# jzombie/rust-simd-r-drive

Hardware: AMD Instinct MI355X
Metric: GiB/s hashed (device-resident), full-file validate+index scan (higher is better)
Workload: dtype u8

## Files before the change

include/srd_amd.h:

```cpp
#ifndef SRD_AMD_H
#define SRD_AMD_H
#include <stddef.h>
#include <stdint.h>

#ifdef __cplusplus
extern "C" {
#endif

#define SRD_OK 0
#define SRD_ERR_HIP (-1)
#define SRD_ERR_ALLOC (-2)
#define SRD_ERR_ARG (-3)
#define SRD_ERR_INTERNAL (-4)

#define SRD_MODE_OPTIMISTIC 0
#define SRD_MODE_FULL 1
#define SRD_MODE_SPAN_UNPROVEN 3

#define SRD_FULL_NONE 0
#define SRD_FULL_FORCED 1
#define SRD_FULL_SLOT_SPACE 2
#define SRD_FULL_WAVES 3
#define SRD_FULL_NO_START 4
#define SRD_FULL_UNPROVEN 5
#define SRD_FULL_CAP 6
#define SRD_FULL_LOOKBACK 7

#define SRD_FLAG_FORCE_FULL 1u
#define SRD_FLAG_NO_CRC 2u
#define SRD_FLAG_STAGE_PAGEABLE 4u
#define SRD_FLAG_STAGE_REGISTER 8u

typedef struct srd_ctx srd_ctx;

int srd_ctx_create(int device, srd_ctx **out);
void srd_ctx_destroy(srd_ctx *ctx);
void *srd_ctx_stream(srd_ctx *ctx);
uint64_t srd_ctx_device_bytes(srd_ctx *ctx);
int srd_ctx_scan_loads(srd_ctx *ctx);
int srd_ctx_scan_trial(srd_ctx *ctx, double *ms);
#define SRD_SCAN_BLOCKS_LAST 0
#define SRD_SCAN_BLOCKS_NEXT 1
#define SRD_SCAN_BLOCKS_EVEN 0
#define SRD_SCAN_BLOCKS_MEASURED 1
#define SRD_SCAN_BLOCKS_INSTALLED 2
typedef struct {
  uint64_t n_spans;
  uint32_t n_blocks;
  uint32_t source;
  uint32_t attempts;
  uint32_t first_source;
} srd_scan_blocks_info;
int srd_ctx_set_scan_blocks(srd_ctx *ctx, const uint64_t *starts,
                            uint32_t n_blocks, uint64_t n_spans);
int srd_ctx_scan_blocks(srd_ctx *ctx, int which, uint64_t *starts,
                        uint32_t cap, srd_scan_blocks_info *info);
const char *srd_last_error(void);
const char *srd_build_info(void);
#define SRD_TIMING_NONE 0
#define SRD_TIMING_SCAN 1
#define SRD_TIMING_CALL 2
int srd_ctx_set_timing(srd_ctx *ctx, int level);
// ... 324 lines not shown
```

rust-simd-r-drive_amd/csrc/srd_ctx.hip:

```cpp
static thread_local std::string g_err;
static void set_err(const std::string& s) { g_err = s; }

#define HIPCHK(x)                                                                         \
  do {                                                                                    \
    hipError_t e_ = (x);                                                                  \
    if (e_ != hipSuccess) {                                                               \
      set_err(std::string(#x) + ": " + hipGetErrorString(e_));                            \
      return SRD_ERR_HIP;                                                                 \
    }                                                                                     \
  } while (0)

namespace {

#define TRY(x)                 \
  do {                         \
    int r_ = (x);              \
    if (r_) return r_;         \
  } while (0)

static int launched(hipStream_t s, const char* name) {
  static const bool sync = [] { const char* e = getenv("SRD_SYNC_DEBUG"); return e && *e && *e != '0'; }();
  HIPCHK(hipGetLastError());
  if (!sync) return 0;
  hipError_t e = hipStreamSynchronize(s);
// ... 48 lines not shown
  }
  void post(std::function<void()> f) {
    std::lock_guard<std::mutex> lk(mu);
    job = std::move(f);
    has = true;
    cv.notify_all();
  }
  void wait() {
    std::unique_lock<std::mutex> lk(mu);
    cv.wait(lk, [this] { return !has; });
  }
};

struct Ctx {
  int device = 0;
  hipStream_t stream = nullptr;
  std::vector<Buf> bufs;
  CandCap copt{8, 8, 0, 8};
  CandCap cfull{32, 32, 0, 32};
  unsigned scan_blocks = 256;
  unsigned scan_cus = 256;
  uint32_t scan_wq[16] = {};
  uint32_t scan_variant = 0;
  uint64_t slot_limit = 1ull << 31;
  int loads_pin = -1;
  int last_loads = -1;
  struct LoadTune {
    uint64_t ns = ~0ull;
    uint32_t g = 0;
    uint32_t calls = 0;
    uint64_t best[2] = {0, 0};
    uint32_t n[2] = {0, 0};
    int choice = -1;
  } tune;
  bool glue_fused = true;
  uint32_t lb_fail = ~0u;
  bool xpart_on = true, xp_valid = false;
  uint32_t xp_par = 0, xp_g = 0;
  uint64_t xp_ns = 0;
  bool xp_installed = false;
  struct LastPart {
    bool any = false;
    uint64_t ns = 0;
    uint32_t g = 0, src = 0, par = 0;
    uint32_t attempts = 0, first_src = 0;
  } xp_last;
// ... 299 lines not shown
      gs += x;
      q = *end == ',' ? end + 1 : end;
      if (*end && *end != ',') { n = 0; break; }
    }
    if (!std::isfinite(gs)) n = 0;
    if (n == 4)
      for (int v = 0; v < 16; v++) f[v] = g[v / 4];
    else if (n == 16)
      for (int v = 0; v < 16; v++) f[v] = g[v];
  }
  weights_to_shares(f, wq);
}
#ifdef SRD_DEBUG_API
extern "C" int srd_debug_set_scan_variant(srd_ctx* c, int v) {
  if (!c || !(v == 0 || v == 7 || v == 8 || v == SCAN_LINES)) return SRD_ERR_ARG;
  c->scan_variant = (uint32_t)v;
  return 0;
}
extern "C" int srd_debug_set_scan_bpc(srd_ctx* c, int bpc) {
  if (!c || bpc < 1 || bpc > 2) return SRD_ERR_ARG;
  c->scan_blocks = c->scan_cus * (unsigned)bpc;
  return 0;
}
extern "C" int srd_debug_set_xpart(srd_ctx* c, int on) {
  if (!c) return SRD_ERR_ARG;
  c->xpart_on = on != 0;
  return 0;
}
extern "C" int srd_debug_set_glue_fused(srd_ctx* c, int fused) {
  if (!c) return SRD_ERR_ARG;
  c->glue_fused = fused != 0;
  return 0;
}
extern "C" int srd_debug_set_scan_weights(srd_ctx* c, const double* w, int n) {
  if (!c || !w || (n != 4 && n != 16)) return SRD_ERR_ARG;
  double f[16], sum = 0;
  for (int v = 0; v < 16; v++) {
    sum += f[v] = n == 4 ? w[v / 4] : w[v];
    if (!(f[v] > 0) || !std::isfinite(f[v])) return SRD_ERR_ARG;
  }
  if (!std::isfinite(sum)) return SRD_ERR_ARG;
  weights_to_shares(f, c->scan_wq);
  return 0;
}
#endif
static int ctx_init(srd_ctx* c, int device) {
// ... 2 lines not shown
  if (hipStreamCreateWithFlags(&c->stream, hipStreamNonBlocking) != hipSuccess) {
    set_err("hipStreamCreate failed");
    return SRD_ERR_HIP;
  }
  TRY(upload_tables());
  for (auto& e : c->ev) HIPCHK(hipEventCreateWithFlags(&e, hipEventReleaseToDevice));
  HIPCHK(hipEventCreateWithFlags(&c->ev_ready, hipEventDisableTiming));
  HIPCHK(hipHostMalloc((void**)&c->h_plan, sizeof(Plan), hipHostMallocDefault));
  HIPCHK(hipHostMalloc((void**)&c->h_pub, 64, hipHostMallocCoherent));
  memset(c->h_pub, 0, 64);
  HIPCHK(hipHostMalloc((void**)&c->h_small, 256, hipHostMallocDefault));
  c->stage_workers = (int)std::max(1u, std::min(8u, std::thread::hardware_concurrency()));
  int ncu = 0;
  if (hipDeviceGetAttribute(&ncu, hipDeviceAttributeMultiprocessorCount, device) == hipSuccess && ncu > 0)
    c->scan_cus = c->scan_blocks = (unsigned)ncu;
  scan_weights(c->scan_wq);
  if (const char* e = getenv("SRD_SLOT_LIMIT_LOG2")) {
    const long v = strtol(e, nullptr, 10);
    if (v >= 10 && v <= 31) c->slot_limit = 1ull << v;
  }
  if (const char* e = getenv("SRD_SCAN_LOADS")) {
    if (!strcmp(e, "lines")) c->loads_pin = SCAN_LINES;
    else if (!strcmp(e, "coal")) c->loads_pin = 0;
  }
  if (const char* e = getenv("SRD_GLUE_FUSED")) c->glue_fused = strcmp(e, "0") != 0;
  if (const char* e = getenv("SRD_XPART")) c->xpart_on = strcmp(e, "0") != 0;
  if (const char* e = getenv("SRD_LB_FAIL_BLOCK")) {
    char* end = nullptr;
    const unsigned long v = strtoul(e, &end, 10);
    if (end != e && v < CHAIN_BLOCKS) c->lb_fail = (uint32_t)v;
  }
  return 0;
}

extern "C" int srd_ctx_create(int device, srd_ctx** out) {
  if (!out) { set_err("null out"); return SRD_ERR_ARG; }
  int n = 0;
  HIPCHK(hipGetDeviceCount(&n));
  if (device < 0 || device >= n) { set_err("bad device index"); return SRD_ERR_ARG; }
  HIPCHK(hipSetDevice(device));
  auto* c = new srd_ctx();
  const int r = ctx_init(c, device);
  if (r) {
    srd_ctx_destroy(c);
    return r;
  }
// ... 15 lines not shown
    if (e) hipEventDestroy(e);
  if (c->h_plan) hipHostFree(c->h_plan);
  if (c->h_pub) hipHostFree(c->h_pub);
  if (c->h_small) hipHostFree(c->h_small);
  if (c->h_out) hipHostFree(c->h_out);
  for (int i = 0; i < 2; i++) {
    if (c->pin_ent[i]) hipHostFree(c->pin_ent[i]);
    if (c->wev_copied[i]) hipEventDestroy(c->wev_copied[i]);
    if (c->wev_done[i]) hipEventDestroy(c->wev_done[i]);
  }
  if (c->cstream) hipStreamDestroy(c->cstream);
  for (auto p : c->stage_pin)
    if (p) hipHostFree(p);
  for (auto e : c->stage_ev)
    if (e) hipEventDestroy(e);
  for (auto st : c->stage_streams)
    if (st) hipStreamDestroy(st);
  if (c->stream) hipStreamDestroy(c->stream);
  delete c;
}

extern "C" void* srd_ctx_stream(srd_ctx* c) { return c ? (void*)c->stream : nullptr; }
extern "C" int srd_ctx_scan_loads(srd_ctx* c) { return c ? c->last_loads : -1; }
extern "C" int srd_ctx_scan_trial(srd_ctx* c, double* ms) {
  if (!c) return -1;
  if (ms)
    for (int k = 0; k < 2; k++) ms[k] = c->tune.n[k] ? (double)c->tune.best[k] * 1e-5 : 0.0;
  return c->tune.choice;
}
extern "C" int srd_ctx_set_scan_blocks(srd_ctx* c, const uint64_t* starts, uint32_t n_blocks, uint64_t n_spans) {
  if (!c || !starts) { set_err("bad argument"); return SRD_ERR_ARG; }
  if (!c->xpart_on) { set_err("XCD-aware block shares are off on this context (SRD_XPART=0)"); return SRD_ERR_ARG; }
  if (!part_table_ok(starts, n_blocks, n_spans)) {
    set_err("bad argument: not a block-start table of n_blocks blocks over n_spans spans (srd_ctx_set_scan_blocks)");
    return SRD_ERR_ARG;
  }
  HIPCHK(hipSetDevice(c->device));
  TRY(ensure_z(c, B_XPART, sizeof(XPart)));
  HIPCHK(hipMemcpyAsync(&P<XPart>(c, B_XPART)->bs[c->xp_par][0], starts, ((size_t)n_blocks + 1) * 8,
                        hipMemcpyHostToDevice, c->stream));
  HIPCHK(hipStreamSynchronize(c->stream));
  c->xp_valid = true;
  c->xp_installed = true;
  c->xp_ns = n_spans;
  c->xp_g = n_blocks;
  return 0;
// ... 81 lines not shown
```

rust-simd-r-drive_amd/csrc/srd_glue.hip:

```cpp
#pragma once

namespace srd {

#define GST(ptr, val) srd_gst(&(ptr), (val))

struct Plan {
  uint64_t K;
  uint64_t n_chain;
  uint64_t root_t;
  uint64_t start;
  uint64_t n_index;
  uint64_t n_bad;
  uint64_t n_slow;
  uint64_t chain_core;
  uint64_t max_root, top_gap, overflow;
  uint32_t status;
  uint32_t nroot;
  uint32_t troot;
  uint32_t idx_overflow;
  uint32_t idx_alias;
};
constexpr uint32_t ST_NOSTART = 1, ST_SHAPE = 2, ST_ROOTS = 4, ST_OVERFLOW = 16;
constexpr uint64_t NO_NODE = ~0ull;

// ... 588 lines not shown
      if (!FUSED) pl->start = start;
      pl->status = s2;
      pl->chain_core = tot;
      pl->n_chain = s2 ? 0 : a.coff + tot;
    }
  };
  const bool plan_block = FUSED ? blockIdx.x + 1 == gridDim.x : blockIdx.x == 0;
  if (!FUSED && plan_block && threadIdx.x == 0) write_plan(st, total);
  if (FUSED && troot && plan_block && threadIdx.x == 0) write_plan(0, 0);
  if (st && !troot) return;
  __shared__ uint32_t s_vcnt[BW_MAX];
  __shared__ uint64_t s_lb[2];
  __shared__ uint32_t s_fail, s_nroot, s_lbok;
  __shared__ unsigned long long s_root_t;
  if constexpr (FUSED) {
    if (!troot) {
      if (threadIdx.x == 0) { s_fail = 0; s_nroot = 0; s_root_t = 0; }
      __syncthreads();
      const uint64_t tag = (uint64_t)a.gen << 32;
      const uint32_t wi = threadIdx.x >> 6, lane = threadIdx.x & 63;
      uint32_t nr = 0;
      bool fail = false;
      constexpr int CR = 4;
      for (uint32_t v = wi; v < a.wpb; v += CHAIN_WAVES) {
        const uint64_t w = (uint64_t)blockIdx.x * a.wpb + v;
        const uint32_t n = w < a.n_waves ? (uint32_t)min(a.wave_total[w] & ~(1ull << 63), a.wcap) : 0u;
        const uint64_t gb = w * a.wcap;
        int64_t c_par = PAR_MISS;
        uint64_t c_cg = 0;
        uint32_t cnt = 0;
        for (uint32_t base = 0; base < n; base += CR * 64) {
          uint64_t g[CR], cg[CR], cp[CR];
          int64_t par[CR], pp[CR];
          bool in[CR], need[CR];
#pragma unroll
          for (int r = 0; r < CR; r++) {
            const uint32_t i = base + (uint32_t)r * 64 + lane;
            in[r] = i < n;
            g[r] = gb + (in[r] ? i : 0u);
            par[r] = a.d_par[g[r]];
            cg[r] = a.childof[g[r]];
          }
          bool any = false;
#pragma unroll
          for (int r = 0; r < CR; r++) {
            const uint32_t i = base + (uint32_t)r * 64 + lane;
            const int64_t l0p = r ? (int64_t)(int32_t)__builtin_amdgcn_readlane((uint32_t)par[r - 1], 63) : c_par;
// ... 83 lines not shown
  }
  if (!FUSED || troot) {
    for (uint32_t k = threadIdx.x; k < nbk; k += blockDim.x) hist[k] = 0;
    fin_lds_words(lt, threadIdx.x, ltw, true);
    __syncthreads();
  }
  GLUE_STAMP(3);
  bool root_slow = false;
  const bool root_block = FUSED && !troot ? root_t != 0 : blockIdx.x == 0;
  if (root_block && a.coff && threadIdx.x == 0) {
    uint64_t kh;
    root_slow = finalize_core<true>(f, 0, NO_REC, -1, root_t, &kh, lt);
    atomicAdd(&hist[idx_bucket(kh, log2_nbk)], 1u);
  }
  uint64_t bend = a.coff + before;
  if (!troot) {
    const uint32_t wi = threadIdx.x >> 6, lane = threadIdx.x & 63;
    const uint64_t lt_mask = (1ull << lane) - 1;
    SlowQueue sq = {wslow[wi], 0, 0};
    if constexpr (FUSED) {
      uint32_t btot = 0;
      for (uint32_t v = 0; v < a.wpb; v++) btot += s_vcnt[v];
      bend += btot;
      for (uint32_t v = wi; v < a.wpb; v += CHAIN_WAVES) {
        const uint64_t w = (uint64_t)blockIdx.x * a.wpb + v;
        const uint32_t n = w < a.n_waves ? (uint32_t)min(a.wave_total[w] & ~(1ull << 63), a.wcap) : 0u;
        const uint64_t gb = w * a.wcap;
        uint32_t voff = 0;
        for (uint32_t u = 0; u < v; u++) voff += s_vcnt[u];
        uint64_t run = a.coff + before + voff;
        sq.run0 = run;
        uint32_t c_fl = F_NO_PARENT, c_suf = 0;
        for (uint32_t base = 0; base < n; base += 64 * FIN_R) {
          bool fl[FIN_R];
          uint64_t gi[FIN_R], kh[FIN_R];
          int64_t par[FIN_R];
          uint32_t psuf[FIN_R], rank[FIN_R];
          FinIn e[FIN_R];
#pragma unroll
          for (int r = 0; r < FIN_R; r++) {
            const uint32_t i = base + (uint32_t)r * 64 + lane;
            gi[r] = gb + (i < n ? i : 0u);
            fl[r] = fin_load_record(a, f, gi[r], i < n, e[r], kh[r], par[r], psuf[r]);
          }
          const uint32_t tot = fin_rank(fl, lt_mask, rank);
          bool any = false, need[FIN_R];
#pragma unroll
// ... 448 lines not shown
```

rust-simd-r-drive_amd/csrc/srd_kernels.hip:

```cpp
#include <hip/hip_runtime.h>
#include <stdint.h>

#include "srd_crc.h"
#include "srd_xxh3.h"
#include "srd_part.h"
#include "srd_fin.h"

namespace srd {


typedef uint32_t u32x4 __attribute__((ext_vector_type(4)));
typedef uint64_t u64x2 __attribute__((ext_vector_type(2)));
typedef uint16_t u16x2 __attribute__((ext_vector_type(2)));

constexpr int SPAN_TILES = 4;
constexpr uint64_t SPAN_BYTES = (uint64_t)TILE * SPAN_TILES;
constexpr int64_t PAR_ROOT = -1;
constexpr int64_t PAR_MISS = -2;

constexpr uint32_t F_NT = 256u, F_ZB = 512u;

struct DevTables {
  uint32_t tab[4][256];
  uint32_t lw[64];
// ... 333 lines not shown
  } else {
    const uint64_t wt = a.wave_total[w - 1] & ~(1ull << 63);
    hp = wt > 0 && wt <= a.wcap;
    gprev = (w - 1) * a.wcap + (hp ? wt - 1 : 0);
  }
  const bool hp2 = r >= 2;
  const uint64_t m = a.c_m[gi], mprev = hp ? a.c_m[gprev] : 0, mprev2 = hp2 ? a.c_m[gi - 2] : 0;
  const u32x4 r0 = a.c_rec[gi];
  const uint64_t p = (uint64_t)r0[0] | ((uint64_t)r0[1] << 32);
  bool node = true, tomb = false;
  if (r0[2] & F_NT) {
    const uint64_t dp = m - p;
    tomb = dp == 1 && (r0[2] & F_ZB);
    node = p >= 20 && p < m && (tomb || dp > prepad64(p));
  }
  const uint64_t mp = p - 20;
  const uint64_t sp2 = (mp + 14) / SPAN_BYTES;
  int64_t par = hp && mprev == mp ? (int64_t)gprev : hp2 && mprev2 == mp ? (int64_t)(gi - 2) : PAR_MISS;
  uint64_t pp = 1;
  const bool res = mp >= a.k_lo * (uint64_t)TILE;
  if (node && par == PAR_MISS && res) pp = ld_u64_unaligned(a.file, p - 12);
  const bool maybe_rec = !res || (pp >= 20 && pp < mp);
  if (node && par == PAR_MISS && maybe_rec && sp2 >= a.part.s_lo && sp2 < a.n_spans) {
    const uint64_t w2 = part_span_wave(a.part, sp2 - a.part.s_lo);
    const uint32_t f2 = a.span_first[sp2];
    const uint32_t n2 = (uint32_t)min<uint64_t>(a.span_count[sp2], a.wcap - min<uint64_t>(f2, a.wcap));
    uint32_t lo = 0, hi = n2;
    const uint64_t* cm = a.c_m + w2 * a.wcap + f2;
    while (lo < hi) {
      const uint32_t mid = (lo + hi) >> 1;
      if (cm[mid] < mp) lo = mid + 1; else hi = mid;
    }
    if (lo < n2 && cm[lo] == mp) par = (int64_t)(w2 * a.wcap + f2 + lo);
  }
  if (!node) {
    par = PAR_MISS;
  } else if (par == PAR_MISS) {
    if (a.span_lo) {
      if (p == a.span_lo) par = PAR_ROOT;
    } else if (p >= 21 && pp == 0) {
      par = PAR_ROOT;
    }
  }
  if (tomb) a.c_rec[gi] = u32x4{r0[0], r0[1], r0[2] | F_TOMB, r0[3]};
  a.d_par[gi] = (int32_t)par;
  if (par >= 0) atomicMax(&a.childof[par], claim_word(a.gen, gi));
}

constexpr uint32_t LINK_WPB = 1;
__device__ void xpart_update(const ScanArgs& a) {
  __shared__ unsigned long long s_sp[8], s_du[8], s_t0, s_t1;
  __shared__ float s_w[8];
  __shared__ double s_pre[256 / 64 + 1];
  XPart* xp = a.xp;
  const ScanPart& p = a.part;
  const uint32_t g = p.g, t = threadIdx.x, lane = t & 63, wv = t >> 6;
  if (t < 8) { s_sp[t] = 0; s_du[t] = 0; }
  if (t == 0) { s_t0 = ~0ull; s_t1 = 0; }
  __syncthreads();
  for (uint32_t b = t; b < g; b += 256) {
    const uint32_t x = xp->xcc[b] & 7u;
    const uint64_t t0 = xp->t0[b], du = xp->dur[b];
    atomicAdd(&s_sp[x], (unsigned long long)(part_block_start(p, b + 1) - part_block_start(p, b)));
    atomicAdd(&s_du[x], (unsigned long long)du);
    atomicMin(&s_t0, (unsigned long long)t0);
    atomicMax(&s_t1, (unsigned long long)(t0 + du));
  }
  __syncthreads();
  if (t == 0) {
    xp->scan_ticks = s_t1 > s_t0 ? s_t1 - s_t0 : 0;
    float sp[8], mean = 0;
    int nx = 0;
    for (int x = 0; x < 8; x++) {
      sp[x] = s_du[x] && s_sp[x] ? (float)s_sp[x] / (float)s_du[x] : 0.f;
      if (sp[x] > 0) { mean += sp[x]; nx++; }
    }
    mean = nx ? mean / nx : 1.f;
    for (int x = 0; x < 8; x++) {
      const float m = sp[x] > 0 ? sp[x] / mean : 1.f, old = xp->w[x];
      float v = old > 0 ? 0.25f * old + 0.75f * m : m;
      v = fminf(fmaxf(v, 1.f - XP_CLAMP), 1.f + XP_CLAMP);
      xp->w[x] = v;
      s_w[x] = v;
    }
  }
  __syncthreads();
  auto q_of = [&](uint32_t b) -> double { return b < g ? (double)s_w[xp->xcc[b] & 7u] : 0.0; };
  double part = 0;
  for (uint32_t b = t; b < g; b += 256) part += q_of(b);
// ... 102 lines not shown
__global__ __launch_bounds__(SCAN_WAVES_V2 * 64) __attribute__((amdgpu_waves_per_eu(4, 4)))
void scan_kernel(ScanArgs a) {
  constexpr int NW = SCAN_WAVES_V2;
  static_assert(V == 0 || V == SCAN_LINES || V == 7 || V == 8, "scan variants: 0, SCAN_LINES, 7, 8");
  constexpr bool COALT = V != SCAN_LINES;
  constexpr bool MEMONLY = V == 7, NOHBM = V == 8;
  uint32_t memonly_acc = 0;
  using Lds = ScanLds;
  __shared__ Lds lds;
  constexpr uint64_t RQ_LANES = 64;
  if (blockIdx.x == 0) {
    for (uint32_t i = threadIdx.x; i < a.n_zero_words; i += blockDim.x) a.zero_words[i] = 0;
    for (uint32_t i = threadIdx.x; i < a.n_zero2; i += blockDim.x) a.zero2[i] = 0;
    if (threadIdx.x == 0 && a.sentinel) *a.sentinel = 0;
    if (!FULL && threadIdx.x == 0) {
      a.k_total[0] = 0;
      a.k_total[1] = 0;
      a.counters[0] = 0;
      a.counters[2] = 0;
    }
  }
  uint64_t xp_t0 = 0;
  if (a.xp && threadIdx.x == 0) xp_t0 = __builtin_amdgcn_s_memrealtime();
#ifdef SRD_WAVE_STAMPS
  if (threadIdx.x == 0) {
    g_wave_stamp[8192 + blockIdx.x] = __builtin_amdgcn_s_memrealtime();
    if (blockIdx.x < 256) g_wave_clk[4096 + blockIdx.x] = __builtin_amdgcn_s_memtime();
    uint32_t xcc, hwid;
    asm volatile("s_getreg_b32 %0, hwreg(HW_REG_XCC_ID)" : "=s"(xcc));
    asm volatile("s_getreg_b32 %0, hwreg(HW_REG_HW_ID)" : "=s"(hwid));
    if (blockIdx.x < 256) g_wave_stamp[8192 + 512 + blockIdx.x] = ((uint64_t)hwid << 32) | xcc;
  }
#endif
  load_crc_lds(lds);
#ifdef SRD_WAVE_STAMPS
  if (threadIdx.x == 0 && blockIdx.x < 256) g_wave_stamp[8192 + 256 + blockIdx.x] = __builtin_amdgcn_s_memrealtime();
#endif

  const int lane = threadIdx.x & 63;
  const int wv = __builtin_amdgcn_readfirstlane(threadIdx.x >> 6);
  uint32_t R[4];
  crc_lane_bases(R, lane);
  const uint8_t* __restrict__ file = a.file;
  const uint64_t flen = a.flen;
  uint32_t* win = lds.win[wv];
  const uint32_t nib_lane = lds_off(lds.nib) + 4u * (lane & 31);
  auto line_crc = [&](const uint32_t (&x)[16]) -> uint32_t { return crc_line4(x, lds, R); };
  auto lane_wt = [&](uint32_t c) -> uint32_t { return lane_weight_or(c, nib_lane); };

  const uint64_t total_waves = (uint64_t)gridDim.x * NW;
  const uint64_t w = (uint64_t)blockIdx.x * NW + wv;
  uint64_t r0, r1;
  part_wave_range(a.part, blockIdx.x, (uint32_t)wv, &r0, &r1);
  uint64_t k0 = (a.part.s_lo + r0) * SPAN_TILES;
  uint64_t k1 = min((a.part.s_lo + r1) * SPAN_TILES, a.n_tiles);
  if (k0 >= k1) k0 = k1 = a.k_lo;

  const uint64_t top = FULL ? 0 : find_top(file, flen, a.m_lo == 0);
  if (!FULL && top == 0) {
    const uint64_t sa = k0 / SPAN_TILES, sb = (k1 + SPAN_TILES - 1) / SPAN_TILES;
    for (uint64_t sp = sa + lane; sp < sb; sp += 64) {
      a.span_count[sp] = 0;
      a.span_first[sp] = 0;
    }
    k0 = k1 = a.k_lo;
  }

  uint32_t count = 0;
  uint64_t wtotal = 0;
  bool ovf = false;
  uint32_t tacc0 = 0, tacc1 = 0, scnt = 0, sfirst = 0;
  bool tg_pend = false, sg_pend = false;
  uint64_t tg_base = 0, sg_base = 0;
  uint32_t tg_par = 0, tg_lo = 0, tg_hi = 0, sg_lo = 0, sg_hi = 0;
  uint32_t rq[10];
#pragma unroll
  for (int i = 0; i < 10; i++) rq[i] = 0;
  uint64_t flushed = 0;
  uint64_t rvalid = 0;

  const uint64_t nohbm_k = (a.part.s_lo + part_block_start(a.part, blockIdx.x)) * SPAN_TILES;
  auto load_tile = [&](uint64_t k, uint32_t (&o)[16]) {
    if constexpr (COALT) {
      const uint8_t* tb = file + (NOHBM ? nohbm_k + (k & 1) : k) * (uint64_t)TILE;
#pragma unroll
      for (int j = 0; j < 4; j++) {
        const u32x4 v = __builtin_nontemporal_load((const u32x4*)(tb + coal_lane_off(lane, j)));
        o[4 * j] = v[0]; o[4 * j + 1] = v[1]; o[4 * j + 2] = v[2]; o[4 * j + 3] = v[3];
      }
      return;
    }
    const u32x4* q = (const u32x4*)(file + k * (uint64_t)TILE + 64ull * lane);
#pragma unroll
    for (int j = 0; j < 4; j++) {
      const u32x4 v = q[j];
      o[4 * j] = v[0]; o[4 * j + 1] = v[1]; o[4 * j + 2] = v[2]; o[4 * j + 3] = v[3];
    }
  };

  const uint32_t hb = a.filt_hb;
  uint64_t rootmax = 0;
  {
    uint32_t pl[16];
    const bool has_prev = k0 > a.k_lo;
// ... 1054 lines not shown
```

rust-simd-r-drive_amd/csrc/srd_part.h:

```cpp
#pragma once
#include <stdint.h>

#if defined(__HIPCC__) || defined(__CUDACC__)
#define SRD_PART_HD __host__ __device__ __forceinline__
#else
#define SRD_PART_HD inline
#endif

namespace srd {

struct ScanPart {
  uint64_t s_lo;
  uint64_t ns;
  uint32_t g;
  uint32_t nw;
  uint32_t wq[16];
  uint32_t cw[17];
  const uint64_t* bs;
};

constexpr uint32_t XP_MAX_BLOCKS = 1024;
SRD_PART_HD uint64_t part_table_block_bound(uint64_t ns, uint64_t g) { return (ns * 5 + 4 * g - 1) / (4 * g) + 1; }
SRD_PART_HD bool part_table_ok(const uint64_t* st, uint64_t g, uint64_t ns) {
  if (!st || g < 1 || g > XP_MAX_BLOCKS || st[0] != 0 || st[g] != ns) return false;
  const uint64_t bound = part_table_block_bound(ns, g);
  for (uint64_t b = 0; b < g; b++)
    if (st[b + 1] < st[b] || st[b + 1] - st[b] > bound) return false;
  return true;
}

SRD_PART_HD void part_fill_cw(ScanPart& p) {
  p.cw[0] = 0;
  for (uint32_t v = 0; v < 16; v++) p.cw[v + 1] = p.cw[v] + (v < p.nw ? p.wq[v] : 0u);
}
SRD_PART_HD uint64_t part_cw(const ScanPart& p, uint32_t v) { return p.cw[v]; }
SRD_PART_HD uint64_t part_block_start(const ScanPart& p, uint64_t b) {
  if (p.bs) return p.bs[b];
  return b * p.ns / p.g;
}
SRD_PART_HD void part_wave_range(const ScanPart& p, uint64_t b, uint32_t v, uint64_t* r0, uint64_t* r1) {
  const uint64_t bs = part_block_start(p, b), nb = part_block_start(p, b + 1) - bs;
  *r0 = bs + ((nb * part_cw(p, v)) >> 16);
  *r1 = bs + ((nb * part_cw(p, v + 1)) >> 16);
}
SRD_PART_HD uint64_t part_span_wave(const ScanPart& p, uint64_t rel) {
  uint64_t b;
  if (p.bs) {
    uint64_t lo = 0, hi = p.g - 1;
    while (lo < hi) {
      const uint64_t mid = (lo + hi + 1) >> 1;
      if (p.bs[mid] <= rel) lo = mid; else hi = mid - 1;
    }
    b = lo;
  } else {
    b = rel * p.g / p.ns;
    while (b + 1 < p.g && part_block_start(p, b + 1) <= rel) b++;
  }
  const uint64_t bs = part_block_start(p, b), nb = part_block_start(p, b + 1) - bs, o = rel - bs;
  uint32_t v = 0;
#pragma unroll
  for (uint32_t j = 1; j < 16; j++) v += j < p.nw && o >= ((nb * part_cw(p, j)) >> 16) ? 1u : 0u;
  return b * p.nw + v;
}
SRD_PART_HD uint64_t part_max_wave_spans(const ScanPart& p, bool xpart = false) {
  if (!p.g) return 1;
  uint32_t wmax = 0;
  for (uint32_t v = 0; v < p.nw; v++) wmax = p.wq[v] > wmax ? p.wq[v] : wmax;
  const uint64_t nb = xpart ? part_table_block_bound(p.ns, p.g) : (p.ns + p.g - 1) / p.g;
  return (nb * wmax + 65535) / 65536 + 1;
}

}
```

rust-simd-r-drive_amd/csrc/srd_scan_host.hip:

```cpp

constexpr uint64_t kWide = 1ull << 40;
constexpr uint64_t kMaxFile = 1ull << 48;
#ifdef SRD_DEBUG_API
constexpr uint32_t kDbgScanOnly = 1u << 30;
#endif
template <bool FULL>
static void launch_scan(unsigned g, const ScanArgs& a, hipStream_t s, hipEvent_t e0 = nullptr,
                        hipEvent_t e1 = nullptr) {
  const dim3 grid(g), block(scan_nw((int)a.variant) * 64);
  if (a.variant == SCAN_LINES) {
    if (a.flen > kWide) hipExtLaunchKernelGGL(scan_kernel<FULL, true, SCAN_LINES>, grid, block, 0, s, e0, e1, 0, a);
    else hipExtLaunchKernelGGL(scan_kernel<FULL, false, SCAN_LINES>, grid, block, 0, s, e0, e1, 0, a);
#ifdef SRD_DEBUG_API
  } else if (a.variant == 7) {
    hipExtLaunchKernelGGL(scan_kernel<FULL, false, 7>, grid, block, 0, s, e0, e1, 0, a);
  } else if (a.variant == 8) {
    hipExtLaunchKernelGGL(scan_kernel<FULL, false, 8>, grid, block, 0, s, e0, e1, 0, a);
#endif
  } else if (e0) {
    if (a.flen > kWide)
      hipExtLaunchKernelGGL(scan_kernel<FULL, true>, grid, block, 0, s, e0, e1, 0, a);
    else
      hipExtLaunchKernelGGL(scan_kernel<FULL, false>, grid, block, 0, s, e0, e1, 0, a);
  } else if (a.flen > kWide) {
// ... 12 lines not shown
  k.grown_cap = k.cap;
  k.grown_bytes = bytes;
}

static unsigned scan_grid(const Ctx* c, uint32_t variant, uint64_t ns, uint32_t* nw) {
  *nw = (uint32_t)scan_nw((int)variant);
  return (unsigned)std::min<uint64_t>((ns + *nw - 1) / *nw, (uint64_t)c->scan_blocks);
}
static ScanPart scan_part(const Ctx* c, uint64_t s_lo, uint64_t ns, unsigned g, uint32_t nw) {
  ScanPart p{};
  p.s_lo = s_lo;
  p.ns = ns;
  p.g = g;
  p.nw = nw;
  if (nw == 16) {
    for (int q = 0; q < 16; q++) p.wq[q] = c->scan_wq[q];
  } else {
    for (uint32_t q = 0; q < nw; q++) p.wq[q] = 65536u / nw;
    p.wq[nw - 1] += 65536u - nw * (65536u / nw);
  }
  part_fill_cw(p);
  return p;
}

static int alloc_scan(Ctx* c, uint64_t n_tiles, uint64_t n_spans, uint32_t cap) {
  const uint64_t slots = n_spans * cap;
  TRY(ensure(c, B_TILE, n_tiles * 16));
  TRY(ensure(c, B_SPAN_COUNT, (n_spans + 1) * 4));
  TRY(ensure(c, B_SPAN_BASE, (n_spans + 1) * 8));
  TRY(ensure(c, B_CM, slots * 8));
  TRY(ensure(c, B_CREC, slots * 32));
  TRY(ensure(c, B_COUNTERS, 8 * 8));
  TRY(ensure(c, B_WALK, sizeof(WalkState)));
  return 0;
}

static u32x4* crec1(Ctx* c) { return P<u32x4>(c, B_CREC) + c->bufs[B_CREC].n / 32; }

static int scan_args(Ctx* c, const uint8_t* d_file, uint64_t flen, uint32_t variant, uint32_t cap, ScanArgs* a) {
  *a = ScanArgs{};
  a->variant = variant;
  a->file = d_file;
  a->flen = flen;
  a->n_tiles = (flen + TILE - 1) / TILE;
  a->n_spans = (a->n_tiles + SPAN_TILES - 1) / SPAN_TILES;
  a->cap = cap;
// ... 50 lines not shown
```

rust-simd-r-drive_amd/csrc/srd_validate.hip:

```cpp

static int wait_publish(Ctx* c, uint64_t* w) {
  const uint32_t seq = c->pub_seq;
  volatile const uint64_t* pub = c->h_pub;
  const auto read = [&] {
    bool ok = true;
    for (int i = 0; i < PUB_WORDS; i++) {
      w[i] = pub[i];
      ok = ok && (uint32_t)(w[i] >> 32) == seq;
    }
    return ok;
  };
  for (uint64_t it = 0;; it++) {
    if (read()) return 0;
    if ((it & 1023) == 1023) {
      const hipError_t e = hipStreamQuery(c->stream);
      if (e == hipSuccess) {
        if (read()) return 0;
        set_err("internal: the glue finished without publishing its outcome");
        return SRD_ERR_INTERNAL;
      }
      if (e != hipErrorNotReady) HIPCHK(e);
    }
  }
}
// ... 247 lines not shown

static int opt_scan(Ctx* c, OptAttempt& o, const ScanPart& part, unsigned g, uint64_t lo, uint64_t k_lo,
                    uint64_t s_lo) {
  ScanArgs& a = o.a;
  TRY(scan_args(c, o.d_file, o.flen, o.var, c->copt.cap, &a));
  a.part = part;
  a.xp = o.xp;
  a.xp_next = c->xp_par ^ 1u;
  a.tile = P<uint32_t>(c, B_TILE) - 4 * k_lo;
  a.span_count = P<uint32_t>(c, B_SPAN_COUNT) - s_lo;
  a.span_first = P<uint32_t>(c, B_SPAN_FIRST) - s_lo;
  a.wcap = o.wcap;
  a.k_lo = k_lo;
  a.m_lo = lo;
  a.zero_words = P<uint32_t>(c, B_PLAN);
  a.n_zero_words = (uint32_t)(sizeof(Plan) / 4);
  a.d_par = P<int32_t>(c, B_DPAR);
  a.childof = P<unsigned long long>(c, B_CHILDOF);
  a.gen = c->gen;
  a.span_lo = lo;
  a.zero2 = index_zero_words(c, o.log2_nbk, &a.n_zero2);
  hipEvent_t e0, e1;
  TRY(next_scan_events(c, &e0, &e1));
  launch_scan<false>(g, a, c->stream, e0, e1);
  LAUNCHED(c->stream, "scan_kernel");
  return 0;
}

static ShapeArgs shape_args(Ctx* c, const OptAttempt& o) {
  ShapeArgs sa{};
  sa.file = o.d_file;
  sa.flen = o.flen;
  sa.Kp = o.a.k_total;
  sa.wave_total = o.a.wave_total;
  sa.wcap = o.wcap;
  sa.n_waves = (uint32_t)o.total_waves;
  sa.wpb = o.wpb;
  sa.n_slots = o.capK;
  sa.coff = o.coff;
  sa.c_m = o.a.c_m;
  sa.d_par = o.a.d_par;
  sa.c_rec = o.a.c_rec;
  sa.childof = P<uint64_t>(c, B_CHILDOF);
  sa.flag = P<uint8_t>(c, B_FLAG);
  sa.part = P<uint32_t>(c, B_PART);
  sa.wpart = P<uint32_t>(c, B_PARTEX);
  sa.counters = P<const unsigned long long>(c, B_COUNTERS);
// ... 114 lines not shown
    o.log2_nbk = index_log2_buckets(n_est);
    uint32_t nw;
    const unsigned g = scan_grid(c, 0, ns_rel, &nw);
    o.var = scan_variant_tune(c, ns_rel, g);
    c->last_loads = o.var == SCAN_LINES ? 1 : o.var == 0 ? 0 : -1;
    ScanPart part = scan_part(c, s_lo, ns_rel, g, nw);
    const bool xpart = c->xpart_on && g <= XP_MAX_BLOCKS;
    o.xp = nullptr;
    if (xpart) {
      TRY(ensure_z(c, B_XPART, sizeof(XPart)));
      o.xp = P<XPart>(c, B_XPART);
      if (c->xp_valid && c->xp_ns == ns_rel && c->xp_g == g) part.bs = &o.xp->bs[c->xp_par][0];
    }
    {
      Ctx::LastPart& l = c->xp_last;
      l.any = true;
      l.ns = ns_rel;
      l.g = g;
      l.par = c->xp_par;
      l.src = !part.bs ? SRD_SCAN_BLOCKS_EVEN : c->xp_installed ? SRD_SCAN_BLOCKS_INSTALLED : SRD_SCAN_BLOCKS_MEASURED;
      l.attempts = attempt + 1;
      if (!attempt) l.first_src = l.src;
    }
    o.total_waves = (uint64_t)g * nw;
    const uint64_t spw = part_max_wave_spans(part, xpart);
    o.wcap = spw * c->copt.cap;
    o.capK = o.total_waves * o.wcap;
    if (o.capK >= c->slot_limit) { out->full_reason = SRD_FULL_SLOT_SPACE; return 0; }
    o.wpb = (uint32_t)((o.total_waves + CHAIN_BLOCKS - 1) / CHAIN_BLOCKS);
    if (o.wpb > BW_MAX) { out->full_reason = SRD_FULL_WAVES; return 0; }
    TRY(alloc_scan(c, nt_rel, std::max<uint64_t>(ns_rel, o.total_waves * spw), c->copt.cap));
    TRY(ensure(c, B_SPAN_FIRST, (ns_rel + 1) * 4));
    TRY(alloc_fast(c, o.capK, o.log2_nbk));
    if (c->gen >= 0xFFFFFFF0u || c->gen == 0) {
      c->gen = 0;
      HIPCHK(hipMemsetAsync(P<void>(c, B_HASCHILD), 0, c->bufs[B_HASCHILD].n, c->stream));
      HIPCHK(hipMemsetAsync(P<void>(c, B_HASCHILD2), 0, c->bufs[B_HASCHILD2].n, c->stream));
      HIPCHK(hipMemsetAsync(P<void>(c, B_CHILDOF), 0, c->bufs[B_CHILDOF].n, c->stream));
    }
    ++c->gen;
    TRY(opt_scan(c, o, part, g, lo, k_lo, s_lo));
#ifdef SRD_DEBUG_API
    if (flags & kDbgScanOnly) {
      HIPCHK(hipStreamSynchronize(c->stream));
      *done = true;
      return 0;
    }
#endif
    link2_kernel<<<(unsigned)((o.total_waves + LINK_WPB - 1) / LINK_WPB), 256 * LINK_WPB, 0, c->stream>>>(
// ... 226 lines not shown
```

rust-simd-r-drive_amd/srd_amd.py:

```python
from __future__ import annotations

import ctypes as C
import mmap as _mmap
import os
import subprocess
import time

import numpy as np

HERE = os.path.dirname(os.path.abspath(__file__))
LIB_PATH = os.environ.get("SRD_LIB_PATH") or os.path.join(HERE, "build", "libsrd_amd.so")

SRD_FLAG_FORCE_FULL = 1
SRD_FLAG_NO_CRC = 2
SRD_FLAG_STAGE_PAGEABLE = 4
SRD_FLAG_STAGE_REGISTER = 8
STAGE_MODES = {0: "pinned input", 1: "registered mapping", 2: "bounce buffers", 3: "pageable copy"}
TIMING_NONE, TIMING_SCAN, TIMING_CALL = 0, 1, 2
SRD_MODE_OPTIMISTIC = 0
SRD_MODE_FULL = 1
SRD_MODE_SPAN_UNPROVEN = 3
SRD_FULL_NONE, SRD_FULL_FORCED, SRD_FULL_SLOT_SPACE, SRD_FULL_WAVES = 0, 1, 2, 3
SRD_FULL_NO_START, SRD_FULL_UNPROVEN, SRD_FULL_CAP, SRD_FULL_LOOKBACK = 4, 5, 6, 7
SRD_ERR_ARG, SRD_ERR_FULL = -3, -5
SCAN_BLOCKS_LAST, SCAN_BLOCKS_NEXT = 0, 1
SCAN_BLOCKS_EVEN, SCAN_BLOCKS_MEASURED, SCAN_BLOCKS_INSTALLED = 0, 1, 2
SRD_FLAG_MERGE_INDEX = 16
SRD_MULTI_COMPOSED, SRD_MULTI_NEIGHBOUR, SRD_MULTI_WHOLE_FILE = 0, 1, 2
SPAN_ALIGN = 16384
METADATA_SIZE = 20
NULL_BYTE = b"\x00"
TAG_BITS = 16
OFFSET_MASK = (1 << 48) - 1

EXPORTS = [
    "srd_ctx_create", "srd_ctx_destroy", "srd_ctx_stream", "srd_ctx_device_bytes", "srd_ctx_scan_loads",
    "srd_ctx_scan_trial", "srd_ctx_set_scan_blocks", "srd_ctx_scan_blocks",
    "srd_last_error", "srd_build_info",
    "srd_ctx_timings",
    "srd_ctx_set_timing",
    "srd_validate_index_device", "srd_validate_index", "srd_result_free",
    "srd_recover_valid_chain", "srd_key_indexer_build", "srd_crc32_batch",
    "srd_crc32_batch_device", "srd_xxh3_64_batch", "srd_xxh3_64_batch_device",
    "srd_synth_store_device", "srd_selftest_host", "srd_padded_size",
    "srd_validate_span_device", "srd_index_partition_device", "srd_index_build_device",
    "srd_synth_span_device", "srd_batch_layout", "srd_batch_write", "srd_batch_write_device",
    "srd_index_table_bytes", "srd_index_table_build_device", "srd_index_get_packed_device",
    "srd_batch_read_hashed_device", "srd_batch_read",
    "srd_iter_entries_device", "srd_estimate_compaction_savings_device", "srd_compact_device",
    "srd_shard_cuts", "srd_validate_index_multi", "srd_ctx_stage_info", "srd_index_hash_device",
    "srd_validate_index_multi_device", "srd_ctx_multi_summary", "srd_ctx_scan_list", "srd_ctx_set_timing_every",
    "srd_stream_probe_device", "srd_ctx_multi_shard_ms",
    "srd_index_table_apply_device", "srd_index_table_export_device", "srd_batch_delete_hashed_device",
    "srd_payload_gather_device", "srd_batch_append_device", "srd_compact_live_device",
    "srd_batch_append_segments_device", "srd_payload_scatter_device",
    "srd_namespace_hash_batch_device", "srd_namespace_hash_batch", "srd_ttl_resolve_device",
    "srd_ttl_resolve_keys_device", "srd_ttl_evict_device", "srd_ttl_sweep_device",
    "srd_ctx_reserve_rows", "srd_read_rows_device",
]
# ... 61 lines not shown
def build() -> str:
    subprocess.check_call(["make", "-s", "-C", HERE])
    return LIB_PATH


_lib = None


def lib():
    global _lib
    if _lib is None:
        if not os.path.exists(LIB_PATH):
            raise RuntimeError(f"{LIB_PATH} missing: run `make -C {HERE}` (no CPU fallback exists)")
        try:
            import torch
        except Exception:
            pass
        L = C.CDLL(LIB_PATH)
        vp, u64, u32, i32 = C.c_void_p, C.c_uint64, C.c_uint32, C.c_int
        L.srd_build_info.restype = C.c_char_p
        L.srd_ctx_device_bytes.argtypes = [vp]
        L.srd_ctx_device_bytes.restype = u64
        L.srd_ctx_scan_loads.argtypes = [vp]
        L.srd_ctx_scan_trial.argtypes = [vp, C.POINTER(C.c_double)]
        L.srd_ctx_set_scan_blocks.argtypes = [vp, vp, u32, u64]
        L.srd_ctx_scan_blocks.argtypes = [vp, i32, vp, u32, C.POINTER(ScanBlocksInfo)]
        if not os.environ.get("SRD_LIB_PATH"):
            import importlib.util
            spec = importlib.util.spec_from_file_location("srd_src_hash", os.path.join(HERE, "src_hash.py"))
            sh = importlib.util.module_from_spec(spec)
            spec.loader.exec_module(sh)
            want, got = sh.source_hash(), L.srd_build_info().decode()
            if got != want:
                raise RuntimeError(f"{LIB_PATH} was built from other sources (sha256 {got}, the sources here "
                                   f"{want}): run `make -C {HERE}`")
        L.srd_ctx_create.argtypes = [i32, C.POINTER(vp)]
        L.srd_ctx_destroy.argtypes = [vp]
        L.srd_ctx_stream.argtypes = [vp]
        L.srd_ctx_stream.restype = vp
        L.srd_last_error.restype = C.c_char_p
        L.srd_ctx_timings.argtypes = [vp, C.POINTER(C.c_double), C.POINTER(C.c_int), C.POINTER(C.c_double)]
        L.srd_ctx_set_timing.argtypes = [vp, C.c_int]
        L.srd_ctx_scan_list.argtypes = [vp, C.POINTER(C.c_float), C.c_int]
        L.srd_ctx_set_timing_every.argtypes = [vp, C.c_int]
        L.srd_validate_index_device.argtypes = [vp, vp, u64, u32, C.POINTER(DeviceResult)]
        L.srd_validate_index.argtypes = [vp, vp, u64, u32, C.POINTER(DeviceResult)]
# ... 95 lines not shown
            self.h = C.c_void_p()

    def __del__(self):
        try:
            self.close()
        except Exception:
            pass

    def set_timing(self, level: int):
        _check(lib().srd_ctx_set_timing(self.h, level))

    def set_timing_every(self, n: int):
        _check(lib().srd_ctx_set_timing_every(self.h, n))

    def reserve_rows(self, n: int, row_cap: int) -> None:
        _check(lib().srd_ctx_reserve_rows(self.h, n, row_cap))

    def device_bytes(self) -> int:
        return int(lib().srd_ctx_device_bytes(self.h))

    def scan_loads(self) -> int:
        return int(lib().srd_ctx_scan_loads(self.h))

    def scan_trial(self):
        ms = (C.c_double * 2)()
        ch = int(lib().srd_ctx_scan_trial(self.h, ms))
        return ch, float(ms[0]), float(ms[1])

    def set_scan_blocks(self, starts, n_spans: int):
        st = np.ascontiguousarray(starts, dtype=np.uint64)
        _check(lib().srd_ctx_set_scan_blocks(self.h, C.c_void_p(st.ctypes.data), max(st.size, 1) - 1, n_spans))

    def scan_blocks(self, which: int = SCAN_BLOCKS_LAST):
        info = ScanBlocksInfo()
        _check(lib().srd_ctx_scan_blocks(self.h, which, None, 0, C.byref(info)))
        st = np.zeros(info.n_blocks + 1 if info.n_blocks else 0, np.uint64)
        if st.size:
            _check(lib().srd_ctx_scan_blocks(self.h, which, C.c_void_p(st.ctypes.data), st.size, C.byref(info)))
        return st, info

    def timings(self):
        a, n, b = C.c_double(), C.c_int(), C.c_double()
        _check(lib().srd_ctx_timings(self.h, C.byref(a), C.byref(n), C.byref(b)))
        return a.value, n.value, b.value

    def scan_list(self) -> list[float]:
# ... 1549 lines not shown
```

Before: 4677.

## Add optional split head/tail scan workgroups to rebalance tail spans

Adds an optional mode that launches twice as many scan workgroups, each block's waves split into a head part and a tail part, with tail sizes ramped across block ranks. It is meant to cut straggler time at the end of the scan. The mode is controlled by SRD_SCAN_TAIL, which defaults to off. The glue chain loop also changes from strided to contiguous per-wave assignment, which does run by default. The split mode adds indexing complexity and doubles the wave slots used.

```diff
diff --git a/include/srd_amd.h b/include/srd_amd.h
--- a/include/srd_amd.h
+++ b/include/srd_amd.h
@@ -38,6 +38,7 @@
 void *srd_ctx_stream(srd_ctx *ctx);
 uint64_t srd_ctx_device_bytes(srd_ctx *ctx);
 int srd_ctx_scan_loads(srd_ctx *ctx);
+int srd_ctx_scan_tail(srd_ctx *ctx);
 int srd_ctx_scan_trial(srd_ctx *ctx, double *ms);
 #define SRD_SCAN_BLOCKS_LAST 0
 #define SRD_SCAN_BLOCKS_NEXT 1
diff --git a/rust-simd-r-drive_amd/csrc/srd_ctx.hip b/rust-simd-r-drive_amd/csrc/srd_ctx.hip
--- a/rust-simd-r-drive_amd/csrc/srd_ctx.hip
+++ b/rust-simd-r-drive_amd/csrc/srd_ctx.hip
@@ -94,6 +94,8 @@
   unsigned scan_cus = 256;
   uint32_t scan_wq[16] = {};
   uint32_t scan_variant = 0;
+  int scan_tail = 0;
+  int last_tail = -1;
   uint64_t slot_limit = 1ull << 31;
   int loads_pin = -1;
   int last_loads = -1;
@@ -439,6 +441,11 @@
   c->scan_blocks = c->scan_cus * (unsigned)bpc;
   return 0;
 }
+extern "C" int srd_debug_set_scan_tail(srd_ctx* c, int tail) {
+  if (!c || tail < 0 || tail > (int)PART_TAIL_LIMIT) return SRD_ERR_ARG;
+  c->scan_tail = tail;
+  return 0;
+}
 extern "C" int srd_debug_set_xpart(srd_ctx* c, int on) {
   if (!c) return SRD_ERR_ARG;
   c->xpart_on = on != 0;
@@ -487,6 +494,11 @@
   if (const char* e = getenv("SRD_SCAN_LOADS")) {
     if (!strcmp(e, "lines")) c->loads_pin = SCAN_LINES;
     else if (!strcmp(e, "coal")) c->loads_pin = 0;
+  }
+  if (const char* e = getenv("SRD_SCAN_TAIL")) {
+    char* end = nullptr;
+    const long v = strtol(e, &end, 10);
+    if (end != e && v >= 0 && v <= (long)PART_TAIL_LIMIT) c->scan_tail = (int)v;
   }
   if (const char* e = getenv("SRD_GLUE_FUSED")) c->glue_fused = strcmp(e, "0") != 0;
   if (const char* e = getenv("SRD_XPART")) c->xpart_on = strcmp(e, "0") != 0;
@@ -548,6 +560,7 @@
 
 extern "C" void* srd_ctx_stream(srd_ctx* c) { return c ? (void*)c->stream : nullptr; }
 extern "C" int srd_ctx_scan_loads(srd_ctx* c) { return c ? c->last_loads : -1; }
+extern "C" int srd_ctx_scan_tail(srd_ctx* c) { return c ? c->last_tail : -1; }
 extern "C" int srd_ctx_scan_trial(srd_ctx* c, double* ms) {
   if (!c) return -1;
   if (ms)
diff --git a/rust-simd-r-drive_amd/csrc/srd_glue.hip b/rust-simd-r-drive_amd/csrc/srd_glue.hip
--- a/rust-simd-r-drive_amd/csrc/srd_glue.hip
+++ b/rust-simd-r-drive_amd/csrc/srd_glue.hip
@@ -634,7 +634,8 @@
       uint32_t nr = 0;
       bool fail = false;
       constexpr int CR = 4;
-      for (uint32_t v = wi; v < a.wpb; v += CHAIN_WAVES) {
+      const uint32_t per = (a.wpb + CHAIN_WAVES - 1) / CHAIN_WAVES;
+      for (uint32_t v = wi * per; v < min((wi + 1) * per, a.wpb); v++) {
         const uint64_t w = (uint64_t)blockIdx.x * a.wpb + v;
         const uint32_t n = w < a.n_waves ? (uint32_t)min(a.wave_total[w] & ~(1ull << 63), a.wcap) : 0u;
         const uint64_t gb = w * a.wcap;
@@ -764,7 +765,8 @@
       uint32_t btot = 0;
       for (uint32_t v = 0; v < a.wpb; v++) btot += s_vcnt[v];
       bend += btot;
-      for (uint32_t v = wi; v < a.wpb; v += CHAIN_WAVES) {
+      const uint32_t per = (a.wpb + CHAIN_WAVES - 1) / CHAIN_WAVES;
+      for (uint32_t v = wi * per; v < min((wi + 1) * per, a.wpb); v++) {
         const uint64_t w = (uint64_t)blockIdx.x * a.wpb + v;
         const uint32_t n = w < a.n_waves ? (uint32_t)min(a.wave_total[w] & ~(1ull << 63), a.wcap) : 0u;
         const uint64_t gb = w * a.wcap;
diff --git a/rust-simd-r-drive_amd/csrc/srd_kernels.hip b/rust-simd-r-drive_amd/csrc/srd_kernels.hip
--- a/rust-simd-r-drive_amd/csrc/srd_kernels.hip
+++ b/rust-simd-r-drive_amd/csrc/srd_kernels.hip
@@ -379,7 +379,7 @@
   if (node && par == PAR_MISS && res) pp = ld_u64_unaligned(a.file, p - 12);
   const bool maybe_rec = !res || (pp >= 20 && pp < mp);
   if (node && par == PAR_MISS && maybe_rec && sp2 >= a.part.s_lo && sp2 < a.n_spans) {
-    const uint64_t w2 = part_span_wave(a.part, sp2 - a.part.s_lo);
+    const uint64_t w2 = part_span_wave2(a.part, sp2 - a.part.s_lo);
     const uint32_t f2 = a.span_first[sp2];
     const uint32_t n2 = (uint32_t)min<uint64_t>(a.span_count[sp2], a.wcap - min<uint64_t>(f2, a.wcap));
     uint32_t lo = 0, hi = n2;
@@ -418,10 +418,13 @@
   for (uint32_t b = t; b < g; b += 256) {
     const uint32_t x = xp->xcc[b] & 7u;
     const uint64_t t0 = xp->t0[b], du = xp->dur[b];
-    atomicAdd(&s_sp[x], (unsigned long long)(part_block_start(p, b + 1) - part_block_start(p, b)));
+    atomicAdd(&s_sp[x], (unsigned long long)(part_split(p) ? part_block_head_spans(p, b)
+                                                           : part_block_start(p, b + 1) - part_block_start(p, b)));
     atomicAdd(&s_du[x], (unsigned long long)du);
     atomicMin(&s_t0, (unsigned long long)t0);
     atomicMax(&s_t1, (unsigned long long)(t0 + du));
+    if (part_split(p))
+      atomicMax(&s_t1, (unsigned long long)(xp->t0[g + b] + xp->dur[g + b]));
   }
   __syncthreads();
   if (t == 0) {
@@ -570,9 +573,29 @@
   }
   uint64_t xp_t0 = 0;
   if (a.xp && threadIdx.x == 0) xp_t0 = __builtin_amdgcn_s_memrealtime();
+  const bool split = !FULL && part_split(a.part);
+  const bool tail_wg = split && blockIdx.x >= a.part.g;
+  const uint32_t tblk = tail_wg ? blockIdx.x - a.part.g : blockIdx.x;
+  if (tail_wg && part_tail_spans(a.part, tblk) == 0) {
+    if (threadIdx.x < NW) {
+      const uint64_t we = ((uint64_t)tblk * NW + threadIdx.x) * 2 + 1;
+      a.wave_total[we] = 0;
+      a.wave_root[we] = 0;
+#ifdef SRD_WAVE_STAMPS
+      if (we < 8192) g_wave_stamp[we] = __builtin_amdgcn_s_memrealtime();
+#endif
+    }
+    if (a.xp && threadIdx.x == 0) {
+      a.xp->xcc[blockIdx.x] = 0;
+      a.xp->dur[blockIdx.x] = 0;
+      a.xp->t0[blockIdx.x] = xp_t0;
+    }
+    return;
+  }
 #ifdef SRD_WAVE_STAMPS
   if (threadIdx.x == 0) {
-    g_wave_stamp[8192 + blockIdx.x] = __builtin_amdgcn_s_memrealtime();
+    if (blockIdx.x < 256) g_wave_stamp[8192 + blockIdx.x] = __builtin_amdgcn_s_memrealtime();
+    else if (blockIdx.x < 511) g_wave_stamp[8192 + 768 + blockIdx.x - 256] = __builtin_amdgcn_s_memrealtime();
     if (blockIdx.x < 256) g_wave_clk[4096 + blockIdx.x] = __builtin_amdgcn_s_memtime();
     uint32_t xcc, hwid;
     asm volatile("s_getreg_b32 %0, hwreg(HW_REG_XCC_ID)" : "=s"(xcc));
@@ -597,9 +620,16 @@
   auto lane_wt = [&](uint32_t c) -> uint32_t { return lane_weight_or(c, nib_lane); };
 
   const uint64_t total_waves = (uint64_t)gridDim.x * NW;
-  const uint64_t w = (uint64_t)blockIdx.x * NW + wv;
+  const uint64_t w = split ? ((uint64_t)tblk * NW + wv) * 2 + (tail_wg ? 1u : 0u) : (uint64_t)blockIdx.x * NW + wv;
   uint64_t r0, r1;
-  part_wave_range(a.part, blockIdx.x, (uint32_t)wv, &r0, &r1);
+  if (split) {
+    uint64_t h0, rh, h1;
+    part_wave_head_tail(a.part, tblk, (uint32_t)wv, &h0, &rh, &h1);
+    r0 = tail_wg ? rh : h0;
+    r1 = tail_wg ? h1 : rh;
+  } else {
+    part_wave_range(a.part, blockIdx.x, (uint32_t)wv, &r0, &r1);
+  }
   uint64_t k0 = (a.part.s_lo + r0) * SPAN_TILES;
   uint64_t k1 = min((a.part.s_lo + r1) * SPAN_TILES, a.n_tiles);
   if (k0 >= k1) k0 = k1 = a.k_lo;
@@ -627,7 +657,7 @@
   uint64_t flushed = 0;
   uint64_t rvalid = 0;
 
-  const uint64_t nohbm_k = (a.part.s_lo + part_block_start(a.part, blockIdx.x)) * SPAN_TILES;
+  const uint64_t nohbm_k = (a.part.s_lo + part_block_start(a.part, tblk)) * SPAN_TILES;
   auto load_tile = [&](uint64_t k, uint32_t (&o)[16]) {
     if constexpr (COALT) {
       const uint8_t* tb = file + (NOHBM ? nohbm_k + (k & 1) : k) * (uint64_t)TILE;
diff --git a/rust-simd-r-drive_amd/csrc/srd_part.h b/rust-simd-r-drive_amd/csrc/srd_part.h
--- a/rust-simd-r-drive_amd/csrc/srd_part.h
+++ b/rust-simd-r-drive_amd/csrc/srd_part.h
@@ -17,6 +17,7 @@
   uint32_t wq[16];
   uint32_t cw[17];
   const uint64_t* bs;
+  uint32_t tail_max;
 };
 
 constexpr uint32_t XP_MAX_BLOCKS = 1024;
@@ -62,6 +63,37 @@
   for (uint32_t j = 1; j < 16; j++) v += j < p.nw && o >= ((nb * part_cw(p, j)) >> 16) ? 1u : 0u;
   return b * p.nw + v;
 }
+constexpr uint32_t PART_TAIL_LIMIT = 8;
+SRD_PART_HD bool part_split(const ScanPart& p) { return p.tail_max != 0 && (uint64_t)p.g * 2 <= XP_MAX_BLOCKS; }
+SRD_PART_HD uint64_t part_total_waves(const ScanPart& p) { return (uint64_t)p.g * p.nw * (part_split(p) ? 2u : 1u); }
+SRD_PART_HD uint64_t part_tail_spans(const ScanPart& p, uint64_t b) {
+  if (!part_split(p)) return 0;
+  const uint64_t nr = ((uint64_t)p.g + 7) / 8, rank = b / 8;
+  return nr > 1 ? (p.tail_max * (nr - 1 - rank) + (nr - 1) / 2) / (nr - 1) : p.tail_max;
+}
+SRD_PART_HD void part_wave_head_tail(const ScanPart& p, uint64_t b, uint32_t v, uint64_t* r0, uint64_t* rh,
+                                     uint64_t* r1) {
+  part_wave_range(p, b, v, r0, r1);
+  const uint64_t n = *r1 - *r0, t = part_tail_spans(p, b);
+  *rh = *r1 - (n ? (t < n - 1 ? t : n - 1) : 0);
+}
+SRD_PART_HD uint64_t part_span_wave2(const ScanPart& p, uint64_t rel) {
+  const uint64_t w = part_span_wave(p, rel);
+  if (!part_split(p)) return w;
+  uint64_t r0, rh, r1;
+  part_wave_head_tail(p, w / p.nw, (uint32_t)(w % p.nw), &r0, &rh, &r1);
+  return 2 * w + (rel >= rh ? 1u : 0u);
+}
+SRD_PART_HD uint64_t part_block_head_spans(const ScanPart& p, uint64_t b) {
+  uint64_t n = 0;
+  for (uint32_t v = 0; v < p.nw; v++) {
+    uint64_t r0, rh, r1;
+    part_wave_head_tail(p, b, v, &r0, &rh, &r1);
+    n += rh - r0;
+  }
+  return n;
+}
+
 SRD_PART_HD uint64_t part_max_wave_spans(const ScanPart& p, bool xpart = false) {
   if (!p.g) return 1;
   uint32_t wmax = 0;
diff --git a/rust-simd-r-drive_amd/csrc/srd_scan_host.hip b/rust-simd-r-drive_amd/csrc/srd_scan_host.hip
--- a/rust-simd-r-drive_amd/csrc/srd_scan_host.hip
+++ b/rust-simd-r-drive_amd/csrc/srd_scan_host.hip
@@ -58,6 +58,8 @@
   part_fill_cw(p);
   return p;
 }
+
+static uint32_t scan_tail_for(const Ctx* c) { return c->scan_tail > 0 ? (uint32_t)c->scan_tail : 0u; }
 
 static int alloc_scan(Ctx* c, uint64_t n_tiles, uint64_t n_spans, uint32_t cap) {
   const uint64_t slots = n_spans * cap;
diff --git a/rust-simd-r-drive_amd/csrc/srd_validate.hip b/rust-simd-r-drive_amd/csrc/srd_validate.hip
--- a/rust-simd-r-drive_amd/csrc/srd_validate.hip
+++ b/rust-simd-r-drive_amd/csrc/srd_validate.hip
@@ -293,7 +293,7 @@
   a.zero2 = index_zero_words(c, o.log2_nbk, &a.n_zero2);
   hipEvent_t e0, e1;
   TRY(next_scan_events(c, &e0, &e1));
-  launch_scan<false>(g, a, c->stream, e0, e1);
+  launch_scan<false>(part_split(part) ? 2 * g : g, a, c->stream, e0, e1);
   LAUNCHED(c->stream, "scan_kernel");
   return 0;
 }
@@ -454,9 +454,12 @@
       l.attempts = attempt + 1;
       if (!attempt) l.first_src = l.src;
     }
-    o.total_waves = (uint64_t)g * nw;
     const uint64_t spw = part_max_wave_spans(part, xpart);
     o.wcap = spw * c->copt.cap;
+    part.tail_max = scan_tail_for(c);
+    if (!part_split(part) || part_total_waves(part) * o.wcap >= c->slot_limit) part.tail_max = 0;
+    o.total_waves = part_total_waves(part);
+    c->last_tail = (int)part.tail_max;
     o.capK = o.total_waves * o.wcap;
     if (o.capK >= c->slot_limit) { out->full_reason = SRD_FULL_SLOT_SPACE; return 0; }
     o.wpb = (uint32_t)((o.total_waves + CHAIN_BLOCKS - 1) / CHAIN_BLOCKS);
diff --git a/rust-simd-r-drive_amd/srd_amd.py b/rust-simd-r-drive_amd/srd_amd.py
--- a/rust-simd-r-drive_amd/srd_amd.py
+++ b/rust-simd-r-drive_amd/srd_amd.py
@@ -35,6 +35,7 @@
 
 EXPORTS = [
     "srd_ctx_create", "srd_ctx_destroy", "srd_ctx_stream", "srd_ctx_device_bytes", "srd_ctx_scan_loads",
+    "srd_ctx_scan_tail",
     "srd_ctx_scan_trial", "srd_ctx_set_scan_blocks", "srd_ctx_scan_blocks",
     "srd_last_error", "srd_build_info",
     "srd_ctx_timings",
@@ -142,6 +143,8 @@
         L.srd_ctx_device_bytes.argtypes = [vp]
         L.srd_ctx_device_bytes.restype = u64
         L.srd_ctx_scan_loads.argtypes = [vp]
+        if hasattr(L, "srd_ctx_scan_tail"):
+            L.srd_ctx_scan_tail.argtypes = [vp]
         L.srd_ctx_scan_trial.argtypes = [vp, C.POINTER(C.c_double)]
         L.srd_ctx_set_scan_blocks.argtypes = [vp, vp, u32, u64]
         L.srd_ctx_scan_blocks.argtypes = [vp, i32, vp, u32, C.POINTER(ScanBlocksInfo)]
@@ -283,6 +286,9 @@
     def scan_loads(self) -> int:
         return int(lib().srd_ctx_scan_loads(self.h))
 
+    def scan_tail(self) -> int:
+        return int(lib().srd_ctx_scan_tail(self.h))
+
     def scan_trial(self):
         ms = (C.c_double * 2)()
         ch = int(lib().srd_ctx_scan_trial(self.h, ms))
```

Measured after the change: 4673. Within noise of the previous version (-0.1%).
